# pdishuck/GAVISUNK

Measured on NVIDIA B200. Metric: ont_read_gbp_per_s_sunk_matched_validated, higher is better.
Workload: dtype u64

## Files before the change

### gavisunk_b200/_lib.py

```python
from __future__ import annotations

import ctypes as C
import os

_HERE = os.path.dirname(os.path.abspath(__file__))
LIB_PATH = os.environ.get("GVS_LIB_PATH") or os.path.join(_HERE, "libgavisunk_b200.so")

u8p, u32p, u64p, i32p, i64p, f64p = (C.POINTER(t) for t in (C.c_uint8, C.c_uint32, C.c_uint64, C.c_int32, C.c_int64, C.c_double))
vp = C.c_void_p

PROTOTYPES = {
    "gvs_create": (vp, [C.c_int, C.c_int]),
    "gvs_destroy": (None, [vp]),
    "gvs_last_error": (C.c_char_p, [vp]),
    "gvs_version": (C.c_char_p, []),
    "gvs_set_stream": (C.c_int, [vp, vp]),
    "gvs_sync": (C.c_int, [vp]),
    "gvs_set_profiling": (C.c_int, [vp, C.c_int]),
    "gvs_stage_ms": (C.c_int, [vp, C.c_int, C.POINTER(C.c_float)]),
    "gvs_launch_count": (C.c_uint64, [vp]),
    "gvs_host_alloc": (C.c_int, [C.c_uint64, C.POINTER(vp)]),
    "gvs_host_free": (None, [vp]),
    "gvs_db_load_loc": (C.c_int, [vp, vp, C.c_uint64, vp, vp, vp, vp, C.c_uint64, C.c_uint32]),
    "gvs_db_build": (C.c_int, [vp, vp, vp, C.c_uint32, C.c_int]),
    "gvs_set_probe_variant": (C.c_int, [vp, C.c_int]),
    "gvs_db_size": (C.c_int, [vp, u64p, u64p]),
    "gvs_db_export": (C.c_int, [vp, vp, vp, vp, vp, vp]),
    "gvs_reads_set": (C.c_int, [vp, vp, vp, C.c_uint64, vp, vp, C.c_uint32, C.c_int]),
    "gvs_reads_set_packed": (C.c_int, [vp, vp, vp, C.c_uint64, vp, vp, C.c_uint32, C.c_int]),
    "gvs_set_copy_pipeline": (C.c_int, [vp, C.c_uint64, C.c_uint32]),
    "gvs_set_host_pack": (C.c_int, [vp, C.c_int, C.c_int]),
    "gvs_copy_stats": (C.c_int, [vp, u64p, C.POINTER(C.c_uint32), C.POINTER(C.c_uint32)]),
    "gvs_reads_meta": (C.c_int, [vp, vp, C.c_uint64, vp, vp, C.c_uint32]),
    "gvs_rows_set": (C.c_int, [vp, C.c_int, vp, vp, vp, vp, vp, C.c_uint64, C.c_uint32]),
    "gvs_match": (C.c_int, [vp, u64p]),
    "gvs_rows_get": (C.c_int, [vp, C.c_int, vp, vp, vp, vp, vp]),
    "gvs_diag_filter": (C.c_int, [vp, vp, vp, u64p, u64p]),
    "gvs_best_get": (C.c_int, [vp, vp, vp, vp, vp]),
    "gvs_filter_best": (C.c_int, [vp, vp, u64p]),
    "gvs_contigs_set": (C.c_int, [vp, vp, vp, C.c_uint32]),
    "gvs_group_hist":(C.c_int, [vp, C.c_int, C.POINTER(vp)]),
    "gvs_hist_mode": (C.c_int, [vp, i64p]),
    "gvs_bad_groups": (C.c_int, [vp, i64p, u64p]),
    "gvs_bad_get": (C.c_int, [vp, vp]),
    "gvs_bad_set": (C.c_int, [vp, vp, vp, C.c_uint64, u64p]),
    "gvs_groups_count": (C.c_int, [vp, u64p]),
    "gvs_groups_get": (C.c_int, [vp, vp, vp, vp]),
    "gvs_batches_begin": (C.c_int, [vp]),
    "gvs_batch_stash": (C.c_int, [vp, u64p]),
    "gvs_batches_bind": (C.c_int, [vp, u64p, u64p]),
    "gvs_validate": (C.c_int, [vp, C.c_uint32, u64p]),
    "gvs_pairs_get": (C.c_int, [vp, vp, vp, vp, vp]),
    "gvs_components_local": (C.c_int, [vp, C.POINTER(vp)]),
    "gvs_components_merge_all": (C.c_int, [vp, vp, C.c_uint32, C.c_uint32]),
    "gvs_placements": (C.c_int, [vp, u64p, C.POINTER(vp)]),
    "gvs_placements_get": (C.c_int, [vp, vp, vp, vp, vp, vp, vp]),
    "gvs_support": (C.c_int, [vp, vp, u64p]),
    "gvs_support_get": (C.c_int, [vp, vp, vp, vp, vp]),
    "gvs_intervals": (C.c_int, [vp, u64p]),
    "gvs_intervals_get": (C.c_int, [vp, vp, vp, vp]),
    "gvs_intervals_set": (C.c_int, [vp, vp, vp, vp, C.c_uint64, C.c_uint32]),
    "gvs_gaps": (C.c_int, [vp, vp, u64p, u64p]),
    "gvs_gaps_get": (C.c_int, [vp, vp, vp, vp, vp]),
    "gvs_covprob_table": (C.c_int, [vp, vp, vp, C.c_uint32, C.c_double, C.c_double, vp]),
    "gvs_covprob_gaps": (C.c_int, [vp, vp, vp, C.c_uint64, vp, vp, vp, C.c_uint64, vp, vp, vp]),
    "gvs_slop": (C.c_int, [vp, vp, vp, vp, C.c_uint64, vp, C.c_uint32, C.c_int64]),
    "gvs_synth_assembly": (C.c_int, [vp, vp, vp, C.c_uint32, C.c_double, C.c_double, C.c_uint64]),
    "gvs_synth_reads_plan": (C.c_int, [vp, vp, C.c_uint32, C.c_uint32, C.c_uint64, C.c_double, C.c_double,
                                       C.c_uint32, C.c_uint32, C.c_uint64, vp, u64p]),
    "gvs_synth_reads_fill": (C.c_int, [vp, vp, vp, vp, C.c_uint64]),
}



class FastxStruct(C.Structure):
    _fields_ = [("impl", C.c_void_p), ("seq", C.c_void_p), ("read_off", C.c_void_p), ("names", C.c_void_p),
                ("name_off", C.c_void_p), ("chunk_first", C.c_void_p), ("n_reads", C.c_uint64), ("total_bases", C.c_uint64),
                ("n_files", C.c_uint32), ("pinned", C.c_int), ("words", C.c_void_p), ("n_words", C.c_uint64)]


PROTOTYPES["gvs_fastx_read"] = (C.c_int, [C.POINTER(C.c_char_p), C.c_uint32, C.c_int, C.c_int, C.POINTER(FastxStruct), C.c_char_p,
                                          C.c_uint64])
PROTOTYPES["gvs_fastx_free"] = (None, [C.POINTER(FastxStruct)])
PROTOTYPES["gvs_fastx_pack"] = (C.c_int, [C.POINTER(FastxStruct), C.c_int, C.c_int])
# ... 47 lines not shown
```

### gavisunk_b200/csrc/common.cuh

```cuda
#pragma once
#include <cuda_runtime.h>
#include <stdint.h>
#include <stdio.h>
#include <string.h>

#include <string>
#include <vector>

#include "../../include/gavisunk_b200.h"

typedef uint8_t u8;
typedef uint16_t u16;
typedef uint32_t u32;
typedef uint64_t u64;
typedef int32_t i32;
typedef int64_t i64;

#define GVS_NSM_DEFAULT 148
#define GVS_TILE_BASES 512
#define GVS_SEG_COUNT 16
#define GVS_SEG_COUNT_PACK 48
#define GVS_SEG_MIN_BYTES (256ull << 20)

struct DevBuf {
  void* p = nullptr;
  size_t cap = 0;
  template <typename T>
  T* as() const { return (T*)p; }
};

struct Rows {
  DevBuf read, pos, contig, start, group, gidx;
  u64 n = 0;
};

struct gvs_ctx {
  int device = 0;
  int k = 20;
  int n_sm = GVS_NSM_DEFAULT;
  cudaStream_t stream = 0;
  std::string err;
  u64 launches = 0;
  bool profiling = false;
  cudaEvent_t ev0[GVS_ST_COUNT], ev1[GVS_ST_COUNT];
  bool ev_valid[GVS_ST_COUNT];
  std::vector<void*> pinned;
  cudaStream_t aux[2] = {nullptr, nullptr};
  bool val_attr_set = false;
  int l2_persist_max = -1, l2_window_max = 0;
  size_t l2_carve_set = 0;
  cudaEvent_t ev_fork = nullptr, ev_join[2] = {nullptr, nullptr};

  bool db_ready = false;
  u64 n_loc = 0, n_groups = 0;
  u32 n_contigs = 0;
  DevBuf loc_kmer, loc_contig, loc_start, loc_group, loc_gidx;
  DevBuf loc_pack;
  DevBuf grp_contig, grp_start;
  u64 grp_gen = 0;
  DevBuf tab_keys, tab_rows, tab_kv;
  u64 tab_slots = 0;
  DevBuf filt;
  u64 filt_words = 0;
  bool filt_fp = false;
  int probe_variant = 0;
  DevBuf filt1;
  u64 filt1_words = 0;
  DevBuf contig_hap, contig_hash, contig_len;

  bool reads_ready = false;
  const u8* seq = nullptr;
  bool seq_packed = false;
  const u64* read_off = nullptr;
  u64 n_reads = 0, total_bases = 0;
  DevBuf own_seq, own_off;
  cudaStream_t copy_stream = nullptr;
  cudaEvent_t ev_reads_free = nullptr;
  std::vector<cudaEvent_t> seg_ev;
  std::vector<u64> seg_tile_end;
  u64 seg_min_bytes = GVS_SEG_MIN_BYTES;
  u32 seg_count = GVS_SEG_COUNT;
// ... 379 lines not shown
```

### gavisunk_b200/csrc/diag.cu

```cuda
#include "common.cuh"

#define NOBEST 0xFFFFFFFFu
#define BANDWIDTH 2500

int gvs_build_segments(gvs_ctx* ctx, const u32* read, u64 n, DevBuf& seg_start, DevBuf& row_seg, u64* n_seg_out);

__global__ void __launch_bounds__(256) k_seg_fill(const u32* __restrict__ read, const u32* __restrict__ row_seg, u64 n,
                                                  u32* seg_start, u32 n_seg) {
  u64 j = (u64)blockIdx.x * blockDim.x + threadIdx.x;
  if (j > n) return;
  if (j == n) { seg_start[n_seg] = (u32)n; return; }
  if (j == 0 || read[j] != read[j - 1]) seg_start[row_seg[j]] = (u32)j;
}

int gvs_build_segments(gvs_ctx* ctx, const u32* read, u64 n, DevBuf& seg_start, DevBuf& row_seg, u64* n_seg_out) {
  CKR(gvs_reserve(ctx, row_seg, n * 4));
  u32* rs = row_seg.as<u32>();
  u32* tot = (u32*)(ctx->counters.as<u64>() + 8);
  auto f = [read] __device__(u64 j) -> u32 { return (j == 0 || read[j] != read[j - 1]) ? 1u : 0u; };
  auto g = [rs] __device__(u64 j, u32 ex, u32 v) { rs[j] = ex + v - 1; };
  CKR((device_scan<u32>(ctx, n, f, g, OpSum(), tot)));
  u32 ns = 0;
  CKR(read_dev(ctx, tot, &ns));
  CKR(gvs_reserve(ctx, seg_start, ((u64)ns + 1) * 4));
  LAUNCH(k_seg_fill, (unsigned)cdiv(n + 1, 256), 256, 0, read, rs, n, seg_start.as<u32>(), ns);
  *n_seg_out = ns;
  return 0;
}

__device__ __forceinline__ u32 chunk_of_read(const u64* __restrict__ chunk_first, u32 n_chunks, u32 read) {
  u32 lo = 0, hi = n_chunks;
  while (hi - lo > 1) {
    u32 mid = (lo + hi) >> 1;
    if (chunk_first[mid] <= read) lo = mid; else hi = mid;
  }
  return lo;
}

__global__ void __launch_bounds__(256) k_seg_info(const u32* __restrict__ read, const u32* __restrict__ seg_start, u32 n_seg,
                                                  const u64* __restrict__ chunk_first, const u8* __restrict__ chunk_hap,
                                                  u32 n_chunks, u32* seg_chunk, u8* seg_hap, u32* seg_ndist) {
  u32 s = blockIdx.x * blockDim.x + threadIdx.x;
  if (s >= n_seg) return;
  u32 c = chunk_of_read(chunk_first, n_chunks, read[seg_start[s]]);
  seg_chunk[s] = c;
  seg_hap[s] = chunk_hap[c];
  seg_ndist[s] = 0;
}

__global__ void __launch_bounds__(256) k_row_first(const u32* __restrict__ contig, const u32* __restrict__ row_seg,
                                                   const u32* __restrict__ seg_start, u64 n, u32* row_cnt, u32* seg_ndist) {
  u64 j = (u64)blockIdx.x * blockDim.x + threadIdx.x;
  if (j >= n) return;
  u32 s = row_seg[j];
  u32 a = seg_start[s], b = seg_start[s + 1];
  u32 c = contig[j];
  if ((u32)j > a && contig[j - 1] == c) { row_cnt[j] = 0; return; }
  for (u32 i = a; i + 1 < (u32)j; i++)
    if (contig[i] == c) { row_cnt[j] = 0; return; }
  u32 cnt = 1;
  for (u32 i = (u32)j + 1; i < b; i++) cnt += contig[i] == c;
  row_cnt[j] = cnt;
  atomicAdd(&seg_ndist[s], 1u);
}

__global__ void __launch_bounds__(256) k_cand_gather(const u32* __restrict__ cand_row, const u32* __restrict__ cand_voff,
                                                     u32 n_cand, const u32* __restrict__ contig, const u32* __restrict__ pos,
                                                     const u32* __restrict__ start, const u32* __restrict__ group,
                                                     const u32* __restrict__ row_seg, const u32* __restrict__ seg_start,
                                                     u32* v_pos, u32* v_start, u32* v_group) {
  u32 w = (blockIdx.x * blockDim.x + threadIdx.x) >> 5;
  int lane = threadIdx.x & 31;
  if (w >= n_cand) return;
  u32 j = cand_row[w];
  u32 b = seg_start[row_seg[j] + 1];
  u32 c = contig[j];
  u32 o = cand_voff[w];
  for (u32 base = j; base < b; base += 32) {
    u32 i = base + lane;
    bool m = i < b && contig[i] == c;
    u32 bal = __ballot_sync(0xFFFFFFFFu, m);
    if (m) {
      u32 d = o + __popc(bal & ((1u << lane) - 1));
      v_pos[d] = pos[i];
      v_start[d] = start[i];
      v_group[d] = group[i];
    }
    o += __popc(bal);
  }
}

#define VOTE_WARP_MAX 256
#define VOTE_WARPS 4
__global__ void __launch_bounds__(VOTE_WARPS * 32) k_cand_vote_warp(const u32* __restrict__ cand_row, const u32* __restrict__ cand_voff,
                                                                    u32 n_cand, const u32* __restrict__ row_cnt,
                                                                    const u32* __restrict__ v_pos, const u32* __restrict__ v_start,
// ... 639 lines not shown
```

### gavisunk_b200/csrc/validate_reads.cu

```cuda
#include "common.cuh"

#define VCAP_WARP 64
#define VCAP 512
#define VROW_BYTES 80
#define NOV 0xFFFFFFFFu
#define NOT64 0xFFFFFFFFFFFFFFFFull

#define F_MULTI 1u
#define F_GOOD 2u
#define F_PRES 4u

struct VWork {
  u32 *P, *S, *ID, *G;
  u32 *uP, *uS, *uID, *uG;
  u32 *deg, *rep, *label, *csize, *flags;
  u64 *key, *tv, *ct;
};

__device__ __forceinline__ void vwork_carve(VWork& w, u8* base, u32 cap) {
  u64* q = (u64*)base;
  w.key = q; q += cap;
  w.tv = q; q += cap;
  w.ct = q; q += cap;
  u32* p = (u32*)q;
  w.P = p; p += cap; w.S = p; p += cap; w.ID = p; p += cap; w.G = p; p += cap;
  w.uP = p; p += cap; w.uS = p; p += cap; w.uID = p; p += cap; w.uG = p; p += cap;
  w.deg = p; p += cap; w.rep = p; p += cap; w.label = p; p += cap; w.csize = p; p += cap; w.flags = p; p += cap;
}

__device__ __forceinline__ bool pair_ok(u32 pi, u32 si, u32 pj, u32 sj) {
  u64 ds = si > sj ? si - sj : sj - si;
  u64 dp = pi > pj ? pi - pj : pj - pi;
  return 9 * ds < 10 * dp && 10 * dp < 11 * ds;
}

struct ValParams {
  const u32 *read, *pos, *start, *group, *gidx;
  const u32* seg_start;
  u32 n_seg;
  const u8* bad;
  const u64* read_off;
  const u32* read_len;
  u32 min_len;
  u32* out_id;
  u32* out_gidx;
  u32* seg_cnt;
  u8* orient;
  u32 m_lo, m_hi;
  u8* gscratch;
  u32 big_cap;
  u32* stats;
};

template <int NT, int GROUPS, bool GLOBAL>
__global__ void __launch_bounds__(NT* GROUPS) k_validate(const ValParams V) {
  extern __shared__ __align__(16) u8 smem[];
  __shared__ u32 s_n0[GROUPS], s_n1[GROUPS], s_m[GROUPS], s_kept[GROUPS], s_bestroot[GROUPS], s_flag[GROUPS], s_dup[GROUPS];
  __shared__ u32 s_pmin[GROUPS], s_pmax[GROUPS];
  __shared__ u32 s_up[GROUPS], s_dn[GROUPS];
  __shared__ unsigned long long s_best[GROUPS];
  __shared__ u32 s_wtot[GROUPS][NT / 32];
  const int grp = threadIdx.x / NT;
  const int tid = threadIdx.x % NT;
  auto gsync = [&]() {
    if (NT == 32) __syncwarp(); else __syncthreads();
  };
  VWork w;
  const u32 cap = GLOBAL ? V.big_cap : (NT == 32 ? VCAP_WARP : VCAP);
  if (GLOBAL) vwork_carve(w, V.gscratch + (u64)blockIdx.x * VROW_BYTES * cap, cap);
  else vwork_carve(w, smem + (u64)grp * VROW_BYTES * cap, cap);

  for (u32 s = blockIdx.x * GROUPS + grp; s < V.n_seg; s += gridDim.x * GROUPS) {
    const u32 a = V.seg_start[s], b = V.seg_start[s + 1];
    const u32 mrows = b - a;
    if (mrows <= V.m_lo || mrows > V.m_hi) continue;
    gsync();
    if (tid == 0) { s_m[grp] = 0; s_n0[grp] = 0; s_n1[grp] = 0; s_kept[grp] = 0; s_best[grp] = 0; s_bestroot[grp] = NOV; s_flag[grp] = 0; s_dup[grp] = 0; s_pmin[grp] = 0xFFFFFFFFu; s_pmax[grp] = 0; s_up[grp] = 0; s_dn[grp] = 0; }
    gsync();
    const u32 rd = V.read[a];
    const u32 rlen = V.read_len ? V.read_len[rd] : (u32)(V.read_off[rd + 1] - V.read_off[rd]);
    const bool skip = rlen < V.min_len || mrows < 2;
    if (!skip) {
      u32 kept_so_far = 0;
      for (u32 base = 0; base < mrows; base += NT) {
        const u32 i = base + tid;
        bool keep = false;
        u32 gi = 0;
        if (i < mrows) {
          gi = V.gidx[a + i];
          keep = !(V.bad && V.bad[gi]);
        }
        const u32 bal = __ballot_sync(0xFFFFFFFFu, keep);
        if (NT > 32) {
          if ((tid & 31) == 0) s_wtot[grp][tid >> 5] = __popc(bal);
          gsync();
        }
        u32 before = 0, total = __popc(bal);
        if (NT > 32) {
          total = 0;
          for (int wv = 0; wv < NT / 32; wv++) {
            u32 c = s_wtot[grp][wv];
            before += wv < (tid >> 5) ? c : 0u;
            total += c;
          }
        }
        if (keep) {
          const u32 d = kept_so_far + before + __popc(bal & ((1u << (tid & 31)) - 1));
          w.uP[d] = V.pos[a + i];
// ... 334 lines not shown
        if (NT > 32) {
          total = 0;
          for (int wv = 0; wv < NT / 32; wv++) {
            const u32 c = s_wtot[grp][wv];
            before += wv < (tid >> 5) ? c : 0u;
            total += c;
          }
        }
        if (mem) {
          const u32 rank = done + before + __popc(bal & ((1u << (tid & 31)) - 1));
          V.out_id[a + rank] = w.ID[r];
          V.out_gidx[a + rank] = w.G[r];
        }
        done += total;
        if (NT > 32) gsync();
      }
    } else
    for (u32 r = tid; r < m; r += NT) {
      if ((w.flags[r] & 8u) && w.label[r] == broot) {
        const u64 t = w.tv[w.rep[r]];
        u32 rank = 0;
        for (u32 q = 0; q < m; q++) rank += ((w.flags[q] & 8u) != 0) & (w.label[q] == broot) & (w.tv[w.rep[q]] < t);
        V.out_id[a + rank] = w.ID[r];
        V.out_gidx[a + rank] = w.G[r];
      }
    }
    if (tid == 0) {
      V.seg_cnt[s] = w.csize[broot];
      V.orient[s] = (u8)orient;
    }
  }
}

__global__ void __launch_bounds__(256) k_pairs_compact(const u32* __restrict__ seg_start, const u32* __restrict__ seg_cnt,
                                                       const u32* __restrict__ seg_off, u32 n_seg, const u32* __restrict__ out_id,
                                                       const u32* __restrict__ out_gidx, const u32* __restrict__ read,
                                                       const u32* __restrict__ contig, u32* p_read, u32* p_contig, u32* p_group,
                                                       u32* p_gidx) {
  u32 wv = (blockIdx.x * blockDim.x + threadIdx.x) >> 5;
  int lane = threadIdx.x & 31;
  if (wv >= n_seg) return;
  u32 c = seg_cnt[wv];
  if (!c) return;
  u32 a = seg_start[wv], o = seg_off[wv];
  u32 rd = read[a], ct = contig[a];
  for (u32 i = lane; i < c; i += 32) {
    p_read[o + i] = rd;
    p_contig[o + i] = ct;
    p_group[o + i] = out_id[a + i];
    p_gidx[o + i] = out_gidx[a + i];
  }
}

extern "C" int gvs_validate(gvs_ctx* ctx, uint32_t min_read_len, uint64_t* n_pairs_out) {
  if (!ctx) return GVS_E_ARG;
  if (!ctx->diag_ready) return gvs_fail(ctx, GVS_E_STATE, "gvs_validate before gvs_diag_filter / gvs_rows_set(1)");
  if (!ctx->read_off && !ctx->have_read_len) return gvs_fail(ctx, GVS_E_STATE, "gvs_validate: read lengths unknown");
  CK(cudaSetDevice(ctx->device));
  StageTimer tm(ctx, GVS_ST_VALIDATE);
  ctx->val_ready = false;
  ctx->pl_ready = ctx->sup_ready = false;
  ctx->n_pairs = 0;
  if (n_pairs_out) *n_pairs_out = 0;
  Rows& R = ctx->kept;
  u64 n = R.n;
  if (n == 0) {
    ctx->val_ready = true;
    return 0;
  }
  u64 n_seg = 0;
  CKR(gvs_build_segments(ctx, R.read.as<u32>(), n, ctx->kseg_start, ctx->flags_c, &n_seg));
  ctx->n_kseg = n_seg;
  const u32* seg_start = ctx->kseg_start.as<u32>();
  CKR(gvs_reserve(ctx, ctx->val_scratch, (2 * n + 2 * n_seg + 16) * 4));
  u32* out_id = ctx->val_scratch.as<u32>();
  u32* out_gidx = out_id + n;
  u32* seg_cnt = out_gidx + n;
  u32* seg_off = seg_cnt + n_seg;
  CKR(gvs_reserve(ctx, ctx->seg_orient, n_seg));
  u32* mx_dev = (u32*)(ctx->counters.as<u64>() + 22);
  {
    auto f2 = [seg_start] __device__(u64 s) -> u32 { return seg_start[s + 1] - seg_start[s]; };
    auto g2 = [] __device__(u64 s, u32 ex, u32 v) {};
    CKR((device_scan<u32>(ctx, n_seg, f2, g2, OpMax(), mx_dev)));
  }
  u32 max_m = 0;
  CKR(read_dev(ctx, mx_dev, &max_m));
  u32* stats = (u32*)(ctx->counters.as<u64>() + 23);
  CK(cudaMemsetAsync(stats, 0, 8, ctx->stream));
  ValParams V;
  V.read = R.read.as<u32>(); V.pos = R.pos.as<u32>(); V.start = R.start.as<u32>(); V.group = R.group.as<u32>();
  V.gidx = R.gidx.as<u32>();
  V.seg_start = seg_start; V.n_seg = (u32)n_seg;
  V.bad = ctx->bad_ready ? ctx->bad_flag.as<u8>() : nullptr;
  V.read_off = ctx->read_off; V.read_len = ctx->have_read_len ? ctx->read_len.as<u32>() : nullptr;
  V.min_len = min_read_len;
  V.out_id = out_id; V.out_gidx = out_gidx; V.seg_cnt = seg_cnt; V.orient = ctx->seg_orient.as<u8>();
  V.gscratch = nullptr; V.big_cap = 0; V.stats = stats;
  const size_t sm_warp = (size_t)VROW_BYTES * VCAP_WARP * 8, sm_blk = (size_t)VROW_BYTES * VCAP;
  if (!ctx->val_attr_set) {
    CK(cudaFuncSetAttribute((k_validate<32, 8, false>), cudaFuncAttributeMaxDynamicSharedMemorySize, (int)sm_warp));
    CK(cudaFuncSetAttribute((k_validate<256, 1, false>), cudaFuncAttributeMaxDynamicSharedMemorySize, (int)sm_blk));
    ctx->val_attr_set = true;
  }
  const bool tiers = max_m > VCAP_WARP;
  if (tiers) CKR(gvs_fork(ctx));
  if (max_m > VCAP) {
    u32 blocks = (u32)ctx->n_sm;
    u32 bcap = (max_m + 15) & ~15u;
    CKR(gvs_reserve(ctx, ctx->scan_tmp2, (u64)blocks * VROW_BYTES * bcap));
    V.gscratch = ctx->scan_tmp2.as<u8>();
    V.big_cap = bcap;
    V.m_lo = VCAP; V.m_hi = 0xFFFFFFFFu;
    LAUNCH_ON(ctx->aux[1], (k_validate<1024, 1, true>), blocks, 1024, 0, V);
    V.gscratch = nullptr; V.big_cap = 0;
  }
  if (max_m > VCAP_WARP) {
    V.m_lo = VCAP_WARP; V.m_hi = VCAP;
    u64 grid = n_seg;
    u64 capg = (u64)ctx->n_sm * 5;
    if (grid > capg) grid = capg;
    LAUNCH_ON(ctx->aux[0], (k_validate<256, 1, false>), (unsigned)grid, 256, sm_blk, V);
  }
  {
    V.m_lo = 0; V.m_hi = VCAP_WARP;
    u64 grid = cdiv(n_seg, 8);
    u64 capg = (u64)ctx->n_sm * 5;
    if (grid > capg) grid = capg;
    LAUNCH((k_validate<32, 8, false>), (unsigned)grid, 256, sm_warp, V);
  }
  if (tiers) CKR(gvs_join(ctx));
  u32* tot = (u32*)(ctx->counters.as<u64>() + 25);
  {
    auto f = [seg_cnt] __device__(u64 s) -> u32 { return seg_cnt[s]; };
    auto g = [seg_off] __device__(u64 s, u32 ex, u32 v) { seg_off[s] = ex; };
    CKR((device_scan<u32>(ctx, n_seg, f, g, OpSum(), tot)));
  }
  u32 np = 0;
  CKR(read_dev(ctx, tot, &np));
  CKR(gvs_reserve(ctx, ctx->pair_read, (u64)np * 4));
  CKR(gvs_reserve(ctx, ctx->pair_contig, (u64)np * 4));
  CKR(gvs_reserve(ctx, ctx->pair_group, (u64)np * 4));
  CKR(gvs_reserve(ctx, ctx->pair_gidx, (u64)np * 4));
  if (np)
    LAUNCH(k_pairs_compact, (unsigned)cdiv(n_seg * 32, 256), 256, 0, seg_start, seg_cnt, seg_off, (u32)n_seg, out_id, out_gidx,
           R.read.as<u32>(), R.contig.as<u32>(), ctx->pair_read.as<u32>(), ctx->pair_contig.as<u32>(),
           ctx->pair_group.as<u32>(), ctx->pair_gidx.as<u32>());
  ctx->n_pairs = np;
  ctx->val_ready = true;
  if (n_pairs_out) *n_pairs_out = np;
  return 0;
}

extern "C" int gvs_pairs_get(gvs_ctx* ctx, uint32_t* read_idx, uint32_t* contig, uint32_t* group, uint32_t* group_index) {
  if (!ctx) return GVS_E_ARG;
  if (!ctx->val_ready) return gvs_fail(ctx, GVS_E_STATE, "gvs_pairs_get before gvs_validate");
  CK(cudaSetDevice(ctx->device));
  u64 n = ctx->n_pairs;
  if (n == 0) return 0;
  if (read_idx) CK(cudaMemcpyAsync(read_idx, ctx->pair_read.p, n * 4, cudaMemcpyDeviceToHost, ctx->stream));
  if (contig) CK(cudaMemcpyAsync(contig, ctx->pair_contig.p, n * 4, cudaMemcpyDeviceToHost, ctx->stream));
  if (group) CK(cudaMemcpyAsync(group, ctx->pair_group.p, n * 4, cudaMemcpyDeviceToHost, ctx->stream));
  if (group_index) CK(cudaMemcpyAsync(group_index, ctx->pair_gidx.p, n * 4, cudaMemcpyDeviceToHost, ctx->stream));
  CK(cudaStreamSynchronize(ctx->stream));
  return 0;
}
```

### gavisunk_b200/engine.py

```python
from __future__ import annotations

import ctypes as C
import math
from typing import Dict, List, Optional, Sequence, Tuple

import numpy as np

from . import _lib
from ._lib import GavisunkError, GavisunkKeyError

_LUT = np.zeros(256, dtype=np.uint64)
for _ch, _v in (("A", 0), ("C", 1), ("G", 2), ("T", 3), ("U", 3)):
    _LUT[ord(_ch)] = _v
    _LUT[ord(_ch.lower())] = _v
_LUT[1], _LUT[2], _LUT[3] = 1, 2, 3


def encode_kmers(lines: Sequence[bytes], k: Optional[int] = None) -> np.ndarray:
    if len(lines) == 0:
        return np.zeros(0, dtype=np.uint64)
    if k is None:
        k = len(lines[0])
    if all(len(l) == k for l in lines):
        a = np.frombuffer(b"".join(lines), dtype=np.uint8).reshape(len(lines), k)
# ... 386 lines not shown
        self._ck(self.lib.gvs_bad_groups(self.ctx, lim, C.byref(n)))
        self.n_bad = int(n.value)
        return self.n_bad

    def bad_list(self) -> np.ndarray:
        out = np.zeros(self.n_bad, np.uint32)
        self._ck(self.lib.gvs_bad_get(self.ctx, _ptr(out)))
        return out

    def bad_set(self, contig, group) -> int:
        c = _c(contig, np.uint32)
        g = _c(group, np.uint32)
        n = C.c_uint64()
        self._ck(self.lib.gvs_bad_set(self.ctx, _ptr(c), _ptr(g), len(c), C.byref(n)))
        self.n_bad = int(n.value)
        return self.n_bad

    def groups(self, with_hist: bool = False) -> Dict[str, np.ndarray]:
        n = C.c_uint64()
        self._ck(self.lib.gvs_groups_count(self.ctx, C.byref(n)))
        n = int(n.value)
        out = dict(contig=np.zeros(n, np.uint32), group=np.zeros(n, np.uint32))
        if with_hist:
            out["count"] = np.zeros(n, np.int32)
        self._ck(self.lib.gvs_groups_get(self.ctx, _ptr(out["contig"]), _ptr(out["group"]), _ptr(out.get("count"))))
        return out

    def validate(self, min_read_len: int = 10000) -> int:
        n = C.c_uint64()
        self._ck(self.lib.gvs_validate(self.ctx, min_read_len, C.byref(n)))
        self.n_pairs = int(n.value)
        return self.n_pairs

    def pairs(self, pinned: bool = False) -> Dict[str, np.ndarray]:
        n = self.n_pairs
        out = {c: self._out(f"pairs.{c}", n, np.uint32, pinned) for c in ("read", "contig", "group", "gidx")}
        self._ck(self.lib.gvs_pairs_get(self.ctx, _ptr(out["read"]), _ptr(out["contig"]), _ptr(out["group"]),
                                        _ptr(out["gidx"])))
        return out

    def placements(self, pinned: bool = False) -> Dict[str, np.ndarray]:
        n, p = C.c_uint64(), C.c_void_p()
        self._ck(self.lib.gvs_placements(self.ctx, C.byref(n), C.byref(p)))
        self._diff_ptr = int(p.value or 0)
        n = int(n.value)
        out = {c: self._out(f"placements.{c}", n, np.uint32, pinned) for c in ("read", "contig", "start", "end", "n_ids")}
        out["strand"] = self._out("placements.strand", n, np.uint8, pinned)
        self._ck(self.lib.gvs_placements_get(self.ctx, _ptr(out["read"]), _ptr(out["contig"]), _ptr(out["start"]), _ptr(out["end"]),
                                             _ptr(out["n_ids"]), _ptr(out["strand"])))
        return out

    def support(self, contig_len: Sequence[int], allreduce=None) -> Dict[str, np.ndarray]:
        if allreduce is not None:
            allreduce(self._diff_ptr, self.db_groups())
        cl = _c(contig_len, np.uint32)
        n = C.c_uint64()
        self._ck(self.lib.gvs_support(self.ctx, _ptr(cl), C.byref(n)))
        out = {c: np.zeros(int(n.value), np.uint32) for c in ("contig", "start", "end", "depth")}
        self._ck(self.lib.gvs_support_get(self.ctx, _ptr(out["contig"]), _ptr(out["start"]), _ptr(out["end"]), _ptr(out["depth"])))
        return out

    def components_local(self) -> int:
        p = C.c_void_p()
        self._ck(self.lib.gvs_components_local(self.ctx, C.byref(p)))
        return int(p.value or 0)

# ... 107 lines not shown
```

### include/gavisunk_b200.h

```cpp
#ifndef GAVISUNK_B200_H
#define GAVISUNK_B200_H

#include <stdint.h>

#ifdef __cplusplus
extern "C" {
#endif

typedef struct gvs_ctx gvs_ctx;

enum {
  GVS_OK = 0,
  GVS_E_CUDA = -1,
  GVS_E_ARG = -2,
  GVS_E_KEYERROR = -3,
  GVS_E_NOMEM = -4,
  GVS_E_OVERFLOW = -5,
  GVS_E_STATE = -6
};

enum {
  GVS_ST_PROBE = 0,
  GVS_ST_EMIT = 1,
  GVS_ST_DIAG = 2,
// ... 87 lines not shown
                   const uint8_t* chunk_hap, uint32_t n_chunks);
int gvs_rows_set(gvs_ctx* ctx, int which, const uint32_t* read_idx, const uint32_t* pos, const uint32_t* contig,
                 const uint32_t* start, const uint32_t* group, uint64_t n_rows, uint32_t n_contigs);

int gvs_match(gvs_ctx* ctx, uint64_t* n_rows);
int gvs_rows_get(gvs_ctx* ctx, int which, uint32_t* read_idx, uint32_t* pos, uint32_t* contig,
                 uint32_t* start, uint32_t* group);

int gvs_diag_filter(gvs_ctx* ctx, const uint8_t* contig_hap, const uint32_t* contig_hash,
                    uint64_t* n_best, uint64_t* n_kept);
int gvs_best_get(gvs_ctx* ctx, uint32_t* read_idx, uint32_t* contig, uint32_t* ngood,
                 uint8_t* dir);

int gvs_filter_best(gvs_ctx* ctx, const uint32_t* best_contig_of_read, uint64_t* n_kept);

int gvs_contigs_set(gvs_ctx* ctx, const uint8_t* contig_hap, const uint32_t* contig_hash,
                    uint32_t n_contigs);

int gvs_group_hist(gvs_ctx* ctx, int accumulate, int32_t** hist_dev);
int gvs_hist_mode(gvs_ctx* ctx, int64_t mode[2]);
int gvs_bad_groups(gvs_ctx* ctx, const int64_t limit_floor[2], uint64_t* n_bad);
int gvs_bad_get(gvs_ctx* ctx, uint32_t* group_index );
int gvs_bad_set(gvs_ctx* ctx, const uint32_t* contig, const uint32_t* group, uint64_t n, uint64_t* n_bad);
int gvs_groups_count(gvs_ctx* ctx, uint64_t* n_groups);
int gvs_groups_get(gvs_ctx* ctx, uint32_t* contig, uint32_t* group, int32_t* hist);

int gvs_batches_begin(gvs_ctx* ctx);
int gvs_batch_stash(gvs_ctx* ctx, uint64_t* read_base);
int gvs_batches_bind(gvs_ctx* ctx, uint64_t* n_rows, uint64_t* n_reads);

int gvs_validate(gvs_ctx* ctx, uint32_t min_read_len, uint64_t* n_pairs);
int gvs_pairs_get(gvs_ctx* ctx, uint32_t* read_idx, uint32_t* contig, uint32_t* group,
                  uint32_t* group_index);

int gvs_components_local(gvs_ctx* ctx, uint32_t** parent_dev);
int gvs_components_merge_all(gvs_ctx* ctx, const uint32_t* gathered_dev, uint32_t n_ranks, uint32_t own_rank);
int gvs_intervals(gvs_ctx* ctx, uint64_t* n_intervals);
int gvs_intervals_get(gvs_ctx* ctx, uint32_t* contig, uint32_t* start, uint32_t* end);

int gvs_placements(gvs_ctx* ctx, uint64_t* n, int32_t** diff_dev);
int gvs_placements_get(gvs_ctx* ctx, uint32_t* read_idx, uint32_t* contig, uint32_t* start, uint32_t* end, uint32_t* n_ids,
                       uint8_t* strand);
int gvs_support(gvs_ctx* ctx, const uint32_t* contig_len, uint64_t* n_runs);
int gvs_support_get(gvs_ctx* ctx, uint32_t* contig, uint32_t* start, uint32_t* end, uint32_t* depth);

int gvs_intervals_set(gvs_ctx* ctx, const uint32_t* contig, const uint32_t* start, const uint32_t* end,
                      uint64_t n, uint32_t n_contigs);

int gvs_gaps(gvs_ctx* ctx, const uint32_t* contig_len, uint64_t* n_gaps, uint64_t* n_nodata);
int gvs_gaps_get(gvs_ctx* ctx, uint32_t* contig, uint32_t* start, uint32_t* end,
                 uint32_t* nodata_contig);

int gvs_covprob_table(gvs_ctx* ctx, const int64_t* kbp, const int64_t* cnt, uint32_t n_bins,
                      double genome_kbp, double pn, double* table3500);

int gvs_covprob_gaps(gvs_ctx* ctx, const uint32_t* grp_contig, const uint32_t* grp_id, uint64_t n_groups,
                     const uint32_t* gap_contig, const int64_t* gap_start, const int64_t* gap_end,
                     uint64_t n_gaps, const double* table3500, int64_t* max_gap, double* covprob);
int gvs_slop(gvs_ctx* ctx, const uint32_t* contig, int64_t* start, int64_t* end, uint64_t n,
             const uint32_t* contig_len, uint32_t n_contigs, int64_t b);

int gvs_synth_assembly(gvs_ctx* ctx, uint8_t* seq_dev, const uint64_t* contig_len,
                       uint32_t n_contigs_per_hap, double snp_rate, double dup_frac,
                       uint64_t seed);
int gvs_synth_reads_plan(gvs_ctx* ctx, const uint64_t* contig_off_dev, uint32_t contig_lo,
                         uint32_t contig_hi, uint64_t n_reads, double len_mu, double len_sigma,
// ... 10 lines not shown
```

Measured before the change: 396.2.

## Add warp-level fast validate path with tiered forwarding of hard reads

```diff
diff --git a/gavisunk_b200/_lib.py b/gavisunk_b200/_lib.py
--- a/gavisunk_b200/_lib.py
+++ b/gavisunk_b200/_lib.py
@@ -50,6 +50,7 @@
     "gvs_batch_stash": (C.c_int, [vp, u64p]),
     "gvs_batches_bind": (C.c_int, [vp, u64p, u64p]),
     "gvs_validate": (C.c_int, [vp, C.c_uint32, u64p]),
+    "gvs_validate_routes": (C.c_int, [vp, vp]),
     "gvs_pairs_get": (C.c_int, [vp, vp, vp, vp, vp]),
     "gvs_components_local": (C.c_int, [vp, C.POINTER(vp)]),
     "gvs_components_merge_all": (C.c_int, [vp, vp, C.c_uint32, C.c_uint32]),
diff --git a/gavisunk_b200/csrc/common.cuh b/gavisunk_b200/csrc/common.cuh
--- a/gavisunk_b200/csrc/common.cuh
+++ b/gavisunk_b200/csrc/common.cuh
@@ -47,6 +47,7 @@
   std::vector<void*> pinned;
   cudaStream_t aux[2] = {nullptr, nullptr};
   bool val_attr_set = false;
+  int val_fast_blocks = 1;
   int l2_persist_max = -1, l2_window_max = 0;
   size_t l2_carve_set = 0;
   cudaEvent_t ev_fork = nullptr, ev_join[2] = {nullptr, nullptr};
diff --git a/gavisunk_b200/csrc/diag.cu b/gavisunk_b200/csrc/diag.cu
--- a/gavisunk_b200/csrc/diag.cu
+++ b/gavisunk_b200/csrc/diag.cu
@@ -50,18 +50,37 @@
 
 __global__ void __launch_bounds__(256) k_row_first(const u32* __restrict__ contig, const u32* __restrict__ row_seg,
                                                    const u32* __restrict__ seg_start, u64 n, u32* row_cnt, u32* seg_ndist) {
-  u64 j = (u64)blockIdx.x * blockDim.x + threadIdx.x;
-  if (j >= n) return;
-  u32 s = row_seg[j];
-  u32 a = seg_start[s], b = seg_start[s + 1];
-  u32 c = contig[j];
-  if ((u32)j > a && contig[j - 1] == c) { row_cnt[j] = 0; return; }
-  for (u32 i = a; i + 1 < (u32)j; i++)
-    if (contig[i] == c) { row_cnt[j] = 0; return; }
-  u32 cnt = 1;
-  for (u32 i = (u32)j + 1; i < b; i++) cnt += contig[i] == c;
-  row_cnt[j] = cnt;
-  atomicAdd(&seg_ndist[s], 1u);
+  const u32 j = blockIdx.x * blockDim.x + threadIdx.x, lane = threadIdx.x & 31;
+  u32 s = 0, a = 0, b = 0, c = 0;
+  bool head = false;
+  if (j < n) {
+    s = row_seg[j];
+    a = seg_start[s];
+    b = seg_start[s + 1];
+    c = contig[j];
+    head = !(j > a && contig[j - 1] == c);
+    if (!head) row_cnt[j] = 0;
+  }
+  for (u32 H = __ballot_sync(0xFFFFFFFFu, head); H; H &= H - 1) {
+    const u32 src = __ffs(H) - 1;
+    const u32 hj = __shfl_sync(0xFFFFFFFFu, j, src), ha = __shfl_sync(0xFFFFFFFFu, a, src),
+              hb = __shfl_sync(0xFFFFFFFFu, b, src), hc = __shfl_sync(0xFFFFFFFFu, c, src);
+    bool first = true;
+    for (u32 base = ha; base + 1 < hj; base += 32) {
+      const u32 i = base + lane;
+      if (__any_sync(0xFFFFFFFFu, i + 1 < hj && contig[i] == hc)) { first = false; break; }
+    }
+    u32 cnt = 0;
+    if (first)
+      for (u32 base = hj; base < hb; base += 32) {
+        const u32 i = base + lane;
+        cnt += __popc(__ballot_sync(0xFFFFFFFFu, i < hb && contig[i] == hc));
+      }
+    if (lane == src) {
+      row_cnt[hj] = cnt;
+      if (first) atomicAdd(&seg_ndist[s], 1u);
+    }
+  }
 }
 
 __global__ void __launch_bounds__(256) k_cand_gather(const u32* __restrict__ cand_row, const u32* __restrict__ cand_voff,
diff --git a/gavisunk_b200/csrc/validate_reads.cu b/gavisunk_b200/csrc/validate_reads.cu
--- a/gavisunk_b200/csrc/validate_reads.cu
+++ b/gavisunk_b200/csrc/validate_reads.cu
@@ -1,7 +1,9 @@
 #include "common.cuh"
 
 #define VCAP_WARP 64
-#define VCAP 512
+#define VCAP_SMEM 1024
+#define VFAST_CAP 1024
+#define VFAST_WARPS 8
 #define VROW_BYTES 80
 #define NOV 0xFFFFFFFFu
 #define NOT64 0xFFFFFFFFFFFFFFFFull
@@ -46,13 +48,16 @@
   u32* out_gidx;
   u32* seg_cnt;
   u8* orient;
-  u32 m_lo, m_hi;
+  const u32* work;
+  const u32* n_work;
+  u32* fwd;
+  u32* n_fwd;
   u8* gscratch;
   u32 big_cap;
   u32* stats;
 };
 
-template <int NT, int GROUPS, bool GLOBAL>
+template <int NT, int GROUPS, int CAP, bool GLOBAL>
 __global__ void __launch_bounds__(NT* GROUPS) k_validate(const ValParams V) {
   extern __shared__ __align__(16) u8 smem[];
   __shared__ u32 s_n0[GROUPS], s_n1[GROUPS], s_m[GROUPS], s_kept[GROUPS], s_bestroot[GROUPS], s_flag[GROUPS], s_dup[GROUPS];
@@ -66,14 +71,15 @@
     if (NT == 32) __syncwarp(); else __syncthreads();
   };
   VWork w;
-  const u32 cap = GLOBAL ? V.big_cap : (NT == 32 ? VCAP_WARP : VCAP);
+  const u32 cap = GLOBAL ? V.big_cap : CAP;
   if (GLOBAL) vwork_carve(w, V.gscratch + (u64)blockIdx.x * VROW_BYTES * cap, cap);
   else vwork_carve(w, smem + (u64)grp * VROW_BYTES * cap, cap);
 
-  for (u32 s = blockIdx.x * GROUPS + grp; s < V.n_seg; s += gridDim.x * GROUPS) {
+  const u32 n_work = *V.n_work;
+  for (u32 wi = blockIdx.x * GROUPS + grp; wi < n_work; wi += gridDim.x * GROUPS) {
+    const u32 s = V.work[wi];
     const u32 a = V.seg_start[s], b = V.seg_start[s + 1];
     const u32 mrows = b - a;
-    if (mrows <= V.m_lo || mrows > V.m_hi) continue;
     gsync();
     if (tid == 0) { s_m[grp] = 0; s_n0[grp] = 0; s_n1[grp] = 0; s_kept[grp] = 0; s_best[grp] = 0; s_bestroot[grp] = NOV; s_flag[grp] = 0; s_dup[grp] = 0; s_pmin[grp] = 0xFFFFFFFFu; s_pmax[grp] = 0; s_up[grp] = 0; s_dn[grp] = 0; }
     gsync();
@@ -474,6 +480,167 @@
   }
 }
 
+#define VTIERS 6
+__device__ __forceinline__ u32 vtier(u32 mrows) {
+  return mrows <= VCAP_WARP ? 0u : mrows <= 128 ? 1u : mrows <= 256 ? 2u : mrows <= 512 ? 3u : mrows <= VCAP_SMEM ? 4u : 5u;
+}
+
+__device__ __forceinline__ void forward_read(const ValParams& V, u32 s, u32 mrows) {
+  const u32 t = vtier(mrows);
+  V.fwd[(u64)t * V.n_seg + atomicAdd(&V.n_fwd[t], 1u)] = s;
+  if (t == VTIERS - 1) atomicMax(&V.n_fwd[VTIERS], mrows);
+}
+
+#define AJ_NOT_ASC 1u
+#define AJ_NOT_DESC 2u
+#define AJ_ID_GE 4u
+#define AJ_ID_LE 8u
+#define AJ_P_UP 16u
+#define AJ_P_DN 32u
+
+__global__ void __launch_bounds__(VFAST_WARPS * 32) k_validate_fast(const ValParams V) {
+  extern __shared__ __align__(16) u8 smem[];
+  const u32 wv = threadIdx.x >> 5, lane = threadIdx.x & 31;
+  const u32 lt = (1u << lane) - 1;
+  u32* sP = (u32*)smem + wv * 2 * VFAST_CAP;
+  u32* sS = sP + VFAST_CAP;
+  for (u32 s = blockIdx.x * VFAST_WARPS + wv; s < V.n_seg; s += gridDim.x * VFAST_WARPS) {
+    const u32 a = V.seg_start[s], b = V.seg_start[s + 1];
+    const u32 mrows = b - a;
+    const u32 rd = V.read[a];
+    const u32 rlen = V.read_len ? V.read_len[rd] : (u32)(V.read_off[rd + 1] - V.read_off[rd]);
+    if (rlen < V.min_len || mrows < 2) {
+      if (lane == 0) V.seg_cnt[s] = 0;
+      continue;
+    }
+    if (mrows > VFAST_CAP) {
+      if (lane == 0) forward_read(V, s, mrows);
+      continue;
+    }
+    __syncwarp();
+    u32 m = 0, keepm = 0, aj = 0;
+    u32 cP = 0, cS = 0, cI = 0;
+    u32 pmin = 0xFFFFFFFFu, pmax = 0, smin = 0xFFFFFFFFu, smax = 0;
+    for (u32 k = 0, base = 0; base < mrows; base += 32, k++) {
+      const u32 i = base + lane;
+      bool keep = false;
+      u32 p = 0, st = 0, id = 0;
+      if (i < mrows) {
+        keep = !(V.bad && V.bad[V.gidx[a + i]]);
+        if (keep) {
+          p = V.pos[a + i];
+          st = V.start[a + i];
+          id = V.group[a + i];
+        }
+      }
+      const u32 bal = __ballot_sync(0xFFFFFFFFu, keep);
+      const u32 below = bal & lt;
+      const u32 src = below ? 31 - __clz(below) : lane;
+      const u32 xP = __shfl_sync(0xFFFFFFFFu, p, src), xS = __shfl_sync(0xFFFFFFFFu, st, src),
+                xI = __shfl_sync(0xFFFFFFFFu, id, src);
+      if (keep) {
+        const u32 d = m + __popc(below);
+        sP[d] = p;
+        sS[d] = st;
+        if (d > 0) {
+          const u32 qP = below ? xP : cP, qS = below ? xS : cS, qI = below ? xI : cI;
+          aj |= (qS >= st ? AJ_NOT_ASC : 0u) | (qS <= st ? AJ_NOT_DESC : 0u) | (qI >= id ? AJ_ID_GE : 0u) |
+                (qI <= id ? AJ_ID_LE : 0u) | (qP < p ? AJ_P_UP : 0u) | (qP > p ? AJ_P_DN : 0u);
+        }
+        pmin = min(pmin, p);
+        pmax = max(pmax, p);
+        smin = min(smin, st);
+        smax = max(smax, st);
+      }
+      keepm |= (keep ? 1u : 0u) << k;
+      if (bal) {
+        const u32 last = 31 - __clz(bal);
+        cP = __shfl_sync(0xFFFFFFFFu, p, last);
+        cS = __shfl_sync(0xFFFFFFFFu, st, last);
+        cI = __shfl_sync(0xFFFFFFFFu, id, last);
+      }
+      m += __popc(bal);
+    }
+    if (m < 2) {
+      if (lane == 0) V.seg_cnt[s] = 0;
+      continue;
+    }
+    aj = __reduce_or_sync(0xFFFFFFFFu, aj);
+    const u32 mono = !(aj & AJ_NOT_ASC) ? 1u : (!(aj & AJ_NOT_DESC) ? 2u : 0u);
+    const bool dup = mono == 1 ? (aj & AJ_ID_GE) != 0 : (aj & AJ_ID_LE) != 0;
+    const bool steps_up = (aj & (mono == 1 ? AJ_P_UP : AJ_P_DN)) != 0, steps_dn = (aj & (mono == 1 ? AJ_P_DN : AJ_P_UP)) != 0;
+    if (mono == 0 || dup || (steps_up && steps_dn)) {
+      if (lane == 0) forward_read(V, s, mrows);
+      continue;
+    }
+    pmin = __reduce_min_sync(0xFFFFFFFFu, pmin);
+    pmax = __reduce_max_sync(0xFFFFFFFFu, pmax);
+    smin = __reduce_min_sync(0xFFFFFFFFu, smin);
+    smax = __reduce_max_sync(0xFFFFFFFFu, smax);
+    const bool narrow = pmax - pmin < (1u << 28) && smax - smin < (1u << 28);
+    __syncwarp();
+    const u32* P0 = mono == 1 ? sP : sP + (m - 1);
+    const u32* S0 = mono == 1 ? sS : sS + (m - 1);
+    const int step = mono == 1 ? 1 : -1;
+    u32 presm = 0, n_e = 0, lmin = NOV, lmax = 0;
+    auto search = [&](auto ok_fn) {
+      for (u32 k = 0, r = lane; r < m; r += 32, k++) {
+        const u32 pr = P0[step * (int)r], sr = S0[step * (int)r];
+        u32 fp = NOV, fh = NOV;
+        for (u32 q = 0; q < r; q++) {
+          const u32 pq = P0[step * (int)q];
+          if (ok_fn(sr - S0[step * (int)q], pq > pr ? pq - pr : pr - pq)) { fp = q; break; }
+        }
+        for (u32 q = r + 1; q < m; q++) {
+          const u32 pq = P0[step * (int)q];
+          if (ok_fn(S0[step * (int)q] - sr, pq > pr ? pq - pr : pr - pq)) { fh = q; break; }
+        }
+        n_e += fh != NOV;
+        if (fp != NOV || fh != NOV) {
+          presm |= 1u << k;
+          const u32 lab = fp != NOV ? fp : r;
+          lmin = min(lmin, lab);
+          lmax = max(lmax, lab);
+        }
+      }
+    };
+    if (narrow) search([](u32 ds, u32 dp) -> bool { return (9u * ds < 10u * dp) & (10u * dp < 11u * ds); });
+    else search([](u32 ds, u32 dp) -> bool { return (9ull * ds < 10ull * dp) & (10ull * dp < 11ull * ds); });
+    if (__reduce_add_sync(0xFFFFFFFFu, n_e) == 0) {
+      if (lane == 0) V.seg_cnt[s] = 0;
+      continue;
+    }
+    if (__reduce_min_sync(0xFFFFFFFFu, lmin) != __reduce_max_sync(0xFFFFFFFFu, lmax)) {
+      if (lane == 0) forward_read(V, s, mrows);
+      continue;
+    }
+    const u32 npres = __reduce_add_sync(0xFFFFFFFFu, (u32)__popc(presm));
+    u32 kd = 0, done = 0;
+    for (u32 k = 0, base = 0; base < mrows; base += 32, k++) {
+      const u32 i = base + lane;
+      const bool keep = (keepm >> k) & 1u;
+      const u32 kb = __ballot_sync(0xFFFFFFFFu, keep);
+      const u32 d = kd + __popc(kb & lt);
+      const u32 r = mono == 1 ? d : m - 1 - d;
+      const u32 pm = __shfl_sync(0xFFFFFFFFu, presm, r & 31);
+      const bool pres = keep && ((pm >> (r >> 5)) & 1u);
+      const u32 pb = __ballot_sync(0xFFFFFFFFu, pres);
+      if (pres) {
+        const u32 c = done + __popc(pb & lt);
+        const u32 rank = mono == 1 ? c : npres - 1 - c;
+        V.out_id[a + rank] = V.group[a + i];
+        V.out_gidx[a + rank] = V.gidx[a + i];
+      }
+      kd += __popc(kb);
+      done += __popc(pb);
+    }
+    if (lane == 0) {
+      V.seg_cnt[s] = npres;
+      V.orient[s] = steps_dn ? 1 : 0;
+    }
+  }
+}
+
 __global__ void __launch_bounds__(256) k_pairs_compact(const u32* __restrict__ seg_start, const u32* __restrict__ seg_cnt,
                                                        const u32* __restrict__ seg_off, u32 n_seg, const u32* __restrict__ out_id,
                                                        const u32* __restrict__ out_gidx, const u32* __restrict__ read,
@@ -514,22 +681,17 @@
   CKR(gvs_build_segments(ctx, R.read.as<u32>(), n, ctx->kseg_start, ctx->flags_c, &n_seg));
   ctx->n_kseg = n_seg;
   const u32* seg_start = ctx->kseg_start.as<u32>();
-  CKR(gvs_reserve(ctx, ctx->val_scratch, (2 * n + 2 * n_seg + 16) * 4));
+  CKR(gvs_reserve(ctx, ctx->val_scratch, (2 * n + (2 + VTIERS) * n_seg + 16) * 4));
   u32* out_id = ctx->val_scratch.as<u32>();
   u32* out_gidx = out_id + n;
   u32* seg_cnt = out_gidx + n;
   u32* seg_off = seg_cnt + n_seg;
+  u32* fwd = seg_off + n_seg;
   CKR(gvs_reserve(ctx, ctx->seg_orient, n_seg));
-  u32* mx_dev = (u32*)(ctx->counters.as<u64>() + 22);
-  {
-    auto f2 = [seg_start] __device__(u64 s) -> u32 { return seg_start[s + 1] - seg_start[s]; };
-    auto g2 = [] __device__(u64 s, u32 ex, u32 v) {};
-    CKR((device_scan<u32>(ctx, n_seg, f2, g2, OpMax(), mx_dev)));
-  }
-  u32 max_m = 0;
-  CKR(read_dev(ctx, mx_dev, &max_m));
   u32* stats = (u32*)(ctx->counters.as<u64>() + 23);
+  u32* n_fwd = (u32*)(ctx->counters.as<u64>() + 36);
   CK(cudaMemsetAsync(stats, 0, 8, ctx->stream));
+  CK(cudaMemsetAsync(n_fwd, 0, (VTIERS + 1) * 4, ctx->stream));
   ValParams V;
   V.read = R.read.as<u32>(); V.pos = R.pos.as<u32>(); V.start = R.start.as<u32>(); V.group = R.group.as<u32>();
   V.gidx = R.gidx.as<u32>();
@@ -538,40 +700,53 @@
   V.read_off = ctx->read_off; V.read_len = ctx->have_read_len ? ctx->read_len.as<u32>() : nullptr;
   V.min_len = min_read_len;
   V.out_id = out_id; V.out_gidx = out_gidx; V.seg_cnt = seg_cnt; V.orient = ctx->seg_orient.as<u8>();
+  V.work = nullptr; V.n_work = nullptr; V.fwd = fwd; V.n_fwd = n_fwd;
   V.gscratch = nullptr; V.big_cap = 0; V.stats = stats;
-  const size_t sm_warp = (size_t)VROW_BYTES * VCAP_WARP * 8, sm_blk = (size_t)VROW_BYTES * VCAP;
+  const size_t sm_fast = (size_t)8 * VFAST_CAP * VFAST_WARPS;
   if (!ctx->val_attr_set) {
-    CK(cudaFuncSetAttribute((k_validate<32, 8, false>), cudaFuncAttributeMaxDynamicSharedMemorySize, (int)sm_warp));
-    CK(cudaFuncSetAttribute((k_validate<256, 1, false>), cudaFuncAttributeMaxDynamicSharedMemorySize, (int)sm_blk));
+    CK(cudaFuncSetAttribute(k_validate_fast, cudaFuncAttributeMaxDynamicSharedMemorySize, (int)sm_fast));
+    CK(cudaFuncSetAttribute((k_validate<32, 8, VCAP_WARP, false>), cudaFuncAttributeMaxDynamicSharedMemorySize, VROW_BYTES * VCAP_WARP * 8));
+    CK(cudaFuncSetAttribute((k_validate<64, 1, 128, false>), cudaFuncAttributeMaxDynamicSharedMemorySize, VROW_BYTES * 128));
+    CK(cudaFuncSetAttribute((k_validate<128, 1, 256, false>), cudaFuncAttributeMaxDynamicSharedMemorySize, VROW_BYTES * 256));
+    CK(cudaFuncSetAttribute((k_validate<256, 1, 512, false>), cudaFuncAttributeMaxDynamicSharedMemorySize, VROW_BYTES * 512));
+    CK(cudaFuncSetAttribute((k_validate<512, 1, VCAP_SMEM, false>), cudaFuncAttributeMaxDynamicSharedMemorySize, VROW_BYTES * VCAP_SMEM));
+    int per_sm = 0;
+    CK(cudaOccupancyMaxActiveBlocksPerMultiprocessor(&per_sm, k_validate_fast, VFAST_WARPS * 32, sm_fast));
+    ctx->val_fast_blocks = per_sm > 0 ? per_sm : 1;
     ctx->val_attr_set = true;
   }
-  const bool tiers = max_m > VCAP_WARP;
-  if (tiers) CKR(gvs_fork(ctx));
-  if (max_m > VCAP) {
-    u32 blocks = (u32)ctx->n_sm;
-    u32 bcap = (max_m + 15) & ~15u;
+  {
+    u64 grid = cdiv(n_seg, VFAST_WARPS);
+    const u64 capg = (u64)ctx->n_sm * ctx->val_fast_blocks;
+    if (grid > capg) grid = capg;
+    LAUNCH(k_validate_fast, (unsigned)grid, VFAST_WARPS * 32, sm_fast, V);
+  }
+  V.fwd = nullptr; V.n_fwd = nullptr;
+  CKR(gvs_fork(ctx));
+  const unsigned g = (unsigned)ctx->n_sm * 8;
+  auto tier = [&](u32 t) { V.work = fwd + (u64)t * n_seg; V.n_work = n_fwd + t; };
+  tier(4);
+  LAUNCH_ON(ctx->aux[0], (k_validate<512, 1, VCAP_SMEM, false>), (unsigned)ctx->n_sm * 2, 512, VROW_BYTES * VCAP_SMEM, V);
+  tier(3);
+  LAUNCH_ON(ctx->aux[0], (k_validate<256, 1, 512, false>), g, 256, VROW_BYTES * 512, V);
+  tier(2);
+  LAUNCH_ON(ctx->aux[1], (k_validate<128, 1, 256, false>), g, 128, VROW_BYTES * 256, V);
+  tier(1);
+  LAUNCH((k_validate<64, 1, 128, false>), g * 2, 64, VROW_BYTES * 128, V);
+  tier(0);
+  LAUNCH((k_validate<32, 8, VCAP_WARP, false>), g, 256, VROW_BYTES * VCAP_WARP * 8, V);
+  u32 big[2] = {0, 0};
+  CKR(read_dev(ctx, n_fwd + VTIERS - 1, big, 2));
+  if (big[0]) {
+    const u32 blocks = big[0] < (u32)ctx->n_sm ? big[0] : (u32)ctx->n_sm;
+    const u32 bcap = (big[1] + 15) & ~15u;
     CKR(gvs_reserve(ctx, ctx->scan_tmp2, (u64)blocks * VROW_BYTES * bcap));
     V.gscratch = ctx->scan_tmp2.as<u8>();
     V.big_cap = bcap;
-    V.m_lo = VCAP; V.m_hi = 0xFFFFFFFFu;
-    LAUNCH_ON(ctx->aux[1], (k_validate<1024, 1, true>), blocks, 1024, 0, V);
-    V.gscratch = nullptr; V.big_cap = 0;
+    tier(VTIERS - 1);
+    LAUNCH_ON(ctx->aux[1], (k_validate<1024, 1, 0, true>), blocks, 1024, 0, V);
   }
-  if (max_m > VCAP_WARP) {
-    V.m_lo = VCAP_WARP; V.m_hi = VCAP;
-    u64 grid = n_seg;
-    u64 capg = (u64)ctx->n_sm * 5;
-    if (grid > capg) grid = capg;
-    LAUNCH_ON(ctx->aux[0], (k_validate<256, 1, false>), (unsigned)grid, 256, sm_blk, V);
-  }
-  {
-    V.m_lo = 0; V.m_hi = VCAP_WARP;
-    u64 grid = cdiv(n_seg, 8);
-    u64 capg = (u64)ctx->n_sm * 5;
-    if (grid > capg) grid = capg;
-    LAUNCH((k_validate<32, 8, false>), (unsigned)grid, 256, sm_warp, V);
-  }
-  if (tiers) CKR(gvs_join(ctx));
+  CKR(gvs_join(ctx));
   u32* tot = (u32*)(ctx->counters.as<u64>() + 25);
   {
     auto f = [seg_cnt] __device__(u64 s) -> u32 { return seg_cnt[s]; };
@@ -594,6 +769,24 @@
   return 0;
 }
 
+extern "C" int gvs_validate_routes(gvs_ctx* ctx, uint32_t* routes) {
+  if (!ctx || !routes) return GVS_E_ARG;
+  if (!ctx->val_ready) return gvs_fail(ctx, GVS_E_STATE, "gvs_validate_routes before gvs_validate");
+  CK(cudaSetDevice(ctx->device));
+  u32 c[VTIERS] = {}, empty = 0;
+  if (ctx->kept.n) {
+    CKR(read_dev(ctx, (u32*)(ctx->counters.as<u64>() + 36), c, VTIERS));
+    CKR(read_dev(ctx, (u32*)(ctx->counters.as<u64>() + 23), &empty, 1));
+  }
+  const u32 block = c[1] + c[2] + c[3] + c[4];
+  routes[0] = ctx->kept.n ? (u32)ctx->n_kseg - c[0] - block - c[5] : 0u;
+  routes[1] = c[0];
+  routes[2] = block;
+  routes[3] = c[5];
+  routes[4] = empty;
+  return 0;
+}
+
 extern "C" int gvs_pairs_get(gvs_ctx* ctx, uint32_t* read_idx, uint32_t* contig, uint32_t* group, uint32_t* group_index) {
   if (!ctx) return GVS_E_ARG;
   if (!ctx->val_ready) return gvs_fail(ctx, GVS_E_STATE, "gvs_pairs_get before gvs_validate");
diff --git a/gavisunk_b200/engine.py b/gavisunk_b200/engine.py
--- a/gavisunk_b200/engine.py
+++ b/gavisunk_b200/engine.py
@@ -442,6 +442,11 @@
         self.n_pairs = int(n.value)
         return self.n_pairs
 
+    def validate_routes(self) -> Dict[str, int]:
+        out = np.zeros(5, np.uint32)
+        self._ck(self.lib.gvs_validate_routes(self.ctx, _ptr(out)))
+        return dict(zip(("fast", "general_warp", "general_block", "general_global", "empty_graph"), map(int, out)))
+
     def pairs(self, pinned: bool = False) -> Dict[str, np.ndarray]:
         n = self.n_pairs
         out = {c: self._out(f"pairs.{c}", n, np.uint32, pinned) for c in ("read", "contig", "group", "gidx")}
diff --git a/include/gavisunk_b200.h b/include/gavisunk_b200.h
--- a/include/gavisunk_b200.h
+++ b/include/gavisunk_b200.h
@@ -143,6 +143,7 @@
 int gvs_validate(gvs_ctx* ctx, uint32_t min_read_len, uint64_t* n_pairs);
 int gvs_pairs_get(gvs_ctx* ctx, uint32_t* read_idx, uint32_t* contig, uint32_t* group,
                   uint32_t* group_index);
+int gvs_validate_routes(gvs_ctx* ctx, uint32_t* routes);
 
 int gvs_components_local(gvs_ctx* ctx, uint32_t** parent_dev);
 int gvs_components_merge_all(gvs_ctx* ctx, const uint32_t* gathered_dev, uint32_t n_ranks, uint32_t own_rank);
diff --git a/profiles/validate_stage.py b/profiles/validate_stage.py
--- /dev/null
+++ b/profiles/validate_stage.py
@@ -0,0 +1,97 @@
+import argparse
+import json
+import os
+import subprocess
+import sys
+from collections import defaultdict
+
+import numpy as np
+
+ROOT = os.path.dirname(os.path.dirname(os.path.abspath(__file__)))
+sys.path.insert(0, ROOT)
+
+
+def gpu_info():
+    try:
+        out = subprocess.run(["nvidia-smi", "--query-gpu=name,power.limit,clocks.max.sm", "--format=csv,noheader", "-i", "0"],
+                             capture_output=True, text=True, timeout=20).stdout.strip()
+    except Exception as ex:
+        out = f"nvidia-smi unavailable: {ex}"
+    return out
+
+
+def stats(v):
+    v = np.asarray(v, np.float64)
+    return dict(median=round(float(np.median(v)), 3), min=round(float(v.min()), 3), max=round(float(v.max()), 3))
+
+
+def main():
+    ap = argparse.ArgumentParser()
+    ap.add_argument("--reps", type=int, default=20)
+    ap.add_argument("--warmup", type=int, default=2)
+    ap.add_argument("--out", default=None)
+    a = ap.parse_args()
+    import torch
+    from gavisunk_b200 import workload as W
+    from gavisunk_b200.engine import Engine
+    if not torch.cuda.is_available():
+        raise SystemExit("validate_stage.py measures on a GPU; none found")
+    eng = Engine(20)
+    contigs = W.human_contigs(3100.0)
+    wl = W.make_assembly(eng, contigs, snp_rate=1e-3, dup_frac=0.01, seed=1001, name="h3100")
+    W.build_db(eng, wl)
+    batch_args = dict(coverage=3.75, n50=100000.0, sigma=0.8, len_min=1000, len_max=1000000, nchunks=10)
+    batches = [W.new_batch(eng, wl, seed=2001 + 16 * b, **batch_args) for b in range(8)]
+    binds = [(lambda e, b=b: W.bind_batch(e, b)) for b in batches]
+    eng.set_profiling(True)
+    diag = []
+    for i in range(a.warmup + a.reps):
+        per = []
+        eng.run_batches(binds, wl.contig_hap, min_read_len=10000, on_batch=lambda e, b, base: per.append(e.stage_ms("diag")))
+        if i >= a.warmup:
+            diag.append(sum(per))
+    n_pairs = int(eng.n_pairs)
+    val = []
+    for i in range(a.warmup + a.reps):
+        assert eng.validate(10000) == n_pairs
+        if i >= a.warmup:
+            val.append(eng.stage_ms("validate"))
+    from torch.profiler import ProfilerActivity, profile
+    eng.set_profiling(False)
+    torch.cuda.synchronize()
+    with profile(activities=[ProfilerActivity.CUDA]) as prof:
+        eng.run_batches(binds, wl.contig_hap, min_read_len=10000)
+        torch.cuda.synchronize()
+    kern = defaultdict(lambda: [0.0, 0])
+    for e in prof.events():
+        name = e.name
+        if name.startswith("void "):
+            name = name[5:]
+        if not (name.startswith("k_validate") or name.startswith("k_row_first")):
+            continue
+        name = name.split("(")[0]
+        dt = getattr(e, "device_time", None)
+        if dt is None:
+            dt = getattr(e, "cuda_time", 0.0)
+        kern[name][0] += dt / 1e3
+        kern[name][1] += 1
+    if a.out:
+        os.makedirs(a.out, exist_ok=True)
+        with open(os.path.join(a.out, "validate_stage_kernels.txt"), "w") as f:
+            f.write(prof.key_averages().table(sort_by="cuda_time_total", row_limit=40))
+    kept = eng.rows(1)
+    _, rows = np.unique(kept["read"], return_counts=True)
+    tiers = {"le64": int((rows <= 64).sum()), "65_512": int(((rows > 64) & (rows <= 512)).sum()),
+             "513_1024": int(((rows > 512) & (rows <= 1024)).sum()), "gt1024": int((rows > 1024).sum())}
+    routes = eng.validate_routes() if hasattr(eng, "validate_routes") else None
+    print(json.dumps(dict(
+        metric="validate_stage_ms", workload="h3100 (bench.py default: 3.1 Gbp x2, 8 batches of 3.75x, k 20), 1 GPU",
+        gpu=gpu_info(), reps=a.reps, validated_pairs=n_pairs, kept_rows=int(len(kept["read"])), reads_with_rows=int(len(rows)),
+        validate_ms=stats(val), diag_ms_per_run=stats(diag),
+        kernels_ms_per_run={k: dict(ms=round(v[0], 3), launches=v[1]) for k, v in sorted(kern.items())},
+        reads_by_rows=tiers, max_rows=int(rows.max()), routes=routes)))
+    eng.close()
+
+
+if __name__ == "__main__":
+    main()
```

Result: faster. 407.0, median of 6 (+2.7%).
